# pedro-morgado/spatialaudiogen

Hardware: AMD Instinct MI355X
Metric: ambisonic seconds generated/sec (0.1 s windows, 224x448 video) (higher is better)
Workload: dtype f32 (fp32 in / out / accumulate; products on the 16-bit matrix cores with fp32-equivalent operand splits: two fp16 planes (3 products per multiply) for the ResNet trunk's 3x3 convs, whose operand ranges batch-norm bounds, three bf16 planes (6 products) elsewhere - measured against the fp64 oracle as

## Files before the change

spatialaudiogen_amd/csrc/igemm3.hip:

```cpp
#include "igemm3_common.h"

namespace sagen {

template <int BM, int BN, int WM, int WN, int KS, bool PRO>
__device__ __forceinline__ void igemm3_body(const IgemmDesc& d, const int z) {
    constexpr int MT = WM / 32, NT = WN / 32;
    constexpr int WAVES_N = BN / WN, WAVES_M = BM / WM;
    static_assert(WAVES_N * WAVES_M == 4, "4 waves per workgroup");
    constexpr int BK = 16;
    constexpr int NCH = BM >= 64 ? BM / 64 : 1;
    constexpr int NBC = (6 * BN + 255) / 256;
    constexpr int A_PL = BM * 8, B_PL = BN * 8;
    constexpr int SUB_F = 3 * A_PL + 3 * B_PL;
    constexpr int STAGE_F = KS * SUB_F;
    constexpr int NJOB = NBC + NBC + NCH + 3 * NCH;

    __shared__ __attribute__((aligned(16))) float smem[2 * STAGE_F];
    __shared__ RowInfo s_row[BM];
    __shared__ int s_tapb[MAX_TAPS];
    __shared__ __attribute__((aligned(16))) float s_bn[2][MAX_BN_C];

    const int tid = threadIdx.x;
    const int lane = tid & 63;
    const int wave = __builtin_amdgcn_readfirstlane(tid >> 6);
// ... 104 lines not shown
        if (!uni) bad |= (i_kok ^ 1u);
        bad_out = bad;
#ifndef SAGEN_ABLATE_A
        dst = bload16(x_rsrc, (a_voff[c] + i_tb) | (bad << 31));
#endif
    };
    auto load_b = [&](int c, f32x4& dst) {
#ifndef SAGEN_ABLATE_B
        dst = bload16(w_rsrc, (b_voff[c] + i_kbyte) | (i_past << 31));
#endif
    };
    auto store_b = [&](int c, const f32x4& src, float* st) {
#ifndef SAGEN_ABLATE_DSW
        if (NBC * 256 == 6 * BN || b_active[c]) *reinterpret_cast<f32x4*>(st + b_wofs[c]) = src;
#else
        asm volatile("" ::"v"(src));
#endif
    };
    float cv[KS][NCH][4];
    auto convert_job = [&](int ks, int c, int level, const f32x4& src, unsigned bad, int c0, float* st) {
        if (level == 0) {
            f32x4 v = src;
            if (PRO) {
                const int cc = c0 + 4 * kc4;
                const float4 sc = *reinterpret_cast<const float4*>(&s_bn[0][cc]);
                const float4 sh = *reinterpret_cast<const float4*>(&s_bn[1][cc]);
                const bool ok = bad == 0;
                v[0] = ok ? fmaxf(fmaf(v[0], sc.x, sh.x), 0.f) : 0.f;
                v[1] = ok ? fmaxf(fmaf(v[1], sc.y, sh.y), 0.f) : 0.f;
                v[2] = ok ? fmaxf(fmaf(v[2], sc.z, sh.z), 0.f) : 0.f;
                v[3] = ok ? fmaxf(fmaf(v[3], sc.w, sh.w), 0.f) : 0.f;
            }
            cv[ks][c][0] = v[0]; cv[ks][c][1] = v[1]; cv[ks][c][2] = v[2]; cv[ks][c][3] = v[3];
        }
        u32x2 pk;
        pk[0] = split_pair(cv[ks][c][0], cv[ks][c][1]);
        pk[1] = split_pair(cv[ks][c][2], cv[ks][c][3]);
#ifndef SAGEN_ABLATE_DSW
        if (a_active) *reinterpret_cast<u32x2*>(st + level * A_PL + a_wofs[c]) = pk;
#else
        asm volatile("" ::"v"(pk));
#endif
    };

    f32x16 acc[MT][NT];
#pragma unroll
    for (int i = 0; i < MT; ++i)
#pragma unroll
        for (int j = 0; j < NT; ++j)
#pragma unroll
            for (int e = 0; e < 16; ++e) acc[i][j][e] = 0.f;

    const int li = lane & 31, kk = lane >> 5;
    const int foff = 4 * (kk ^ ((li >> 3) & 1));

    auto side_job = [&](int job, int ks, auto pl_tag, float* st) {
        constexpr int PL = decltype(pl_tag)::value, PS = PL ^ 1;
        float* sub = st + ks * SUB_F;
        if (job < NBC) store_b(job, braw[PS][ks][job], sub);
        else if (job < 2 * NBC) load_b(job - NBC, braw[PL][ks][job - NBC]);
        else if (job < 2 * NBC + NCH) load_a(job - 2 * NBC, araw[PL][ks][job - 2 * NBC], abad[PL][ks][job - 2 * NBC]);
        else {
            const int cj = job - 2 * NBC - NCH, c = cj / 3;
            convert_job(ks, c, cj - 3 * c, araw[PS][ks][c], abad[PS][ks][c], ac0[PS][ks], sub);
        }
    };

#ifdef SAGEN_TRACE
    unsigned long long* trc = (d.trace && tile_m == d.trace_block && blockIdx.y == 0) ? (unsigned long long*)d.trace + (size_t)wave * 64 * 8 : nullptr;
#define TRC3(ph) do { if (trc && lane == 0 && t < 64) trc[t * 8 + (ph)] = __builtin_readcyclecounter(); } while (0)
#else
#define TRC3(ph) do { } while (0)
#endif
    constexpr int TA[6] = {0, 0, 1, 0, 2, 1}, TB[6] = {0, 1, 0, 2, 0, 1};
    const int nsteps = (ntiles + KS - 1) / KS;
#pragma unroll
    for (int ks = 0; ks < KS; ++ks) {
        begin_load(kc0 + ks, ac0[0][ks]);
#pragma unroll
        for (int c = 0; c < NBC; ++c) load_b(c, braw[0][ks][c]);
#pragma unroll
        for (int c = 0; c < NCH; ++c) load_a(c, araw[0][ks][c], abad[0][ks][c]);
    }
#pragma unroll
    for (int ks = 0; ks < KS; ++ks) {
        begin_load(kc0 + KS + ks, ac0[1][ks]);
#pragma unroll
        for (int c = 0; c < NBC; ++c) load_b(c, braw[1][ks][c]);
#pragma unroll
        for (int c = 0; c < NCH; ++c) load_a(c, araw[1][ks][c], abad[1][ks][c]);
    }
#pragma unroll
    for (int ks = 0; ks < KS; ++ks) {
#pragma unroll
        for (int c = 0; c < NBC; ++c) store_b(c, braw[0][ks][c], smem + ks * SUB_F);
#pragma unroll
        for (int c = 0; c < NCH; ++c)
#pragma unroll
            for (int lv = 0; lv < 3; ++lv) convert_job(ks, c, lv, araw[0][ks][c], abad[0][ks][c], ac0[0][ks], smem + ks * SUB_F);
    }
    lds_barrier();

    auto step = [&](auto parity, int t) {
        constexpr int P = decltype(parity)::value;
        const float* cur = smem + P * STAGE_F;
        float* nxt = smem + (P ^ 1) * STAGE_F;
            TRC3(0);
#pragma unroll
        for (int ks = 0; ks < KS; ++ks) {
            begin_load(kc0 + (t + 2) * KS + ks, ac0[P][ks]);
            bf16x8 aq[3][MT], bq[3][NT];
#pragma unroll
            for (int pl = 0; pl < 3; ++pl) {
#pragma unroll
                for (int i = 0; i < MT; ++i)
                    aq[pl][i] = *reinterpret_cast<const bf16x8*>(cur + ks * SUB_F + pl * A_PL + (wm * WM + i * 32 + li) * 8 + foff);
#pragma unroll
                for (int j = 0; j < NT; ++j)
                    bq[pl][j] = *reinterpret_cast<const bf16x8*>(cur + ks * SUB_F + 3 * A_PL + pl * B_PL + (wn * WN + j * 32 + li) * 8 + foff);
            }
#pragma unroll
            for (int tt = 0; tt < 6; ++tt)
#pragma unroll
                for (int i = 0; i < MT; ++i)
#pragma unroll
                    for (int j = 0; j < NT; ++j) {
#ifndef SAGEN_ABLATE_MFMA
                        acc[i][j] = __builtin_amdgcn_mfma_f32_32x32x16_bf16(aq[TA[tt]][i], bq[TB[tt]][j], acc[i][j], 0, 0, 0);
#else
                        asm volatile("" ::"v"(aq[TA[tt]][i]), "v"(bq[TB[tt]][j]));
#endif
                        constexpr int NM1 = 6 * MT * NT;
                        const int idx = (tt * MT + i) * NT + j;
#pragma unroll
                        for (int g = 0; g < NJOB; ++g)
                            if (idx == (g * NM1 / NJOB < NM1 ? g * NM1 / NJOB : NM1 - 1)) side_job(g, ks, std::integral_constant<int, P>{}, nxt);
#ifdef SAGEN_TRACE
                        if (ks == 0 && idx == 0) TRC3(1);
                        if (ks == KS - 1 && idx == NM1 - 1) TRC3(2);
#endif
                    }
        }
        asm volatile("s_waitcnt lgkmcnt(0)" ::: "memory");
        TRC3(3);
        lds_barrier();
        TRC3(4);
    };
    for (int t = 0; t < nsteps; t += 2) {
        step(std::integral_constant<int, 0>{}, t);
        if (t + 1 < nsteps) step(std::integral_constant<int, 1>{}, t + 1);
    }

    if (d.mm_out != nullptr) {
        if constexpr (BM <= 128 && BN <= 128 && WM * BN + 7 * 32 <= 2 * STAGE_F && !PRO)
            igemm_epilogue_maskmix<BM, BN, WM, WN, 2 * STAGE_F>(d, acc, smem, m0, n0, tid);
        return;
    }
    if (!igemm_epilogue_rows<BM, BN, WM, WN, 2 * STAGE_F>(d, acc, s_row, smem, n0, tid))
        igemm_epilogue<BM, BN, WM, WN>(d, acc, s_row, smem, m0, n0, z, tid);
}

template <int BM, int BN, int WM, int WN, int KS, bool PRO>
__global__ __launch_bounds__(256, 2) void igemm3_kernel(const IgemmDesc d_in) {
    IgemmDesc d = d_in;
    int z = blockIdx.z;
    if (d.grp.G > 1) {
        const int g = d.splitk == 1 ? z : z / d.splitk;
        z -= g * d.splitk;
        igemm_relocate(d, g);
    }
    igemm3_body<BM, BN, WM, WN, KS, PRO>(d, z);
}

template <int BM, int BN, int WM, int WN, int KS>
static int launch_cfg3(const IgemmDesc& d, hipStream_t s) {
    dim3 grid(cdiv(d.M, BM), cdiv(d.N, BN), d.splitk * d.grp.G);
    if (d.in_scale != nullptr || d.bn_in.acc != nullptr)
        hipLaunchKernelGGL((igemm3_kernel<BM, BN, WM, WN, KS, true>), grid, dim3(256), 0, s, d);
    else
        hipLaunchKernelGGL((igemm3_kernel<BM, BN, WM, WN, KS, false>), grid, dim3(256), 0, s, d);
    SAGEN_LAUNCH_CHECK();
    return SAGEN_OK;
}

int igemm3_dispatch(const IgemmDesc& d, IgemmTile tile, hipStream_t s) {
#define SAGEN_TILE_HAS_B3 ,
    switch (tile) {
        SAGEN_TILES(SAGEN_TILE_CASE)
        default: return igemm3dw_dispatch(d, tile, s);
    }
}

__global__ __launch_bounds__(256) void pack_split_kernel(const float* __restrict__ wp, long total, int N, int Kpad,
                                                         __bf16* __restrict__ w3) {
    const long idx = (long)blockIdx.x * 256 + threadIdx.x;
    if (idx >= total) return;
    const long n = idx / Kpad;
    const int k = (int)(idx - n * Kpad);
    const float v = wp[idx];
    const __bf16 h = (__bf16)v;
    const float r1 = v - (float)h;
    const __bf16 m = (__bf16)r1;
    const float r2 = r1 - (float)m;
    const long o = ((long)(k >> 4) * 3 * N + n) * 16 + (k & 15);
    w3[o] = h; w3[o + (long)N * 16] = m; w3[o + (long)N * 32] = (__bf16)r2;
}

int pack_split_launch(float* wp, int N, int Kpad, hipStream_t s) {
    const long total = (long)N * Kpad;
    hipLaunchKernelGGL(pack_split_kernel, dim3(cdiv(total, 256)), dim3(256), 0, s, wp, total, N, Kpad,
                       reinterpret_cast<__bf16*>(wp + total));
    SAGEN_LAUNCH_CHECK();
    return SAGEN_OK;
}

}
```

spatialaudiogen_amd/csrc/igemm_common.h:

```cpp
#pragma once
#include "kernels.h"
#include "h2_planes.h"

namespace sagen {

typedef float f32x16 __attribute__((ext_vector_type(16)));
constexpr int MAX_TAPS = 128;
constexpr unsigned OOB = 0x80000000u;
constexpr int MAX_BN_C = 512;

struct RowInfo {
    unsigned boff;
    unsigned nmlo, nmhi;
    int hrem, wrem;
    int pad;
    long rowoff;
};

__device__ __forceinline__ void dma16(__amdgpu_buffer_rsrc_t rsrc, float* lds, unsigned voff, unsigned soff) {
#if defined(__HIP_DEVICE_COMPILE__) && !defined(SAGEN_ABLATE_DMA)
    __builtin_amdgcn_raw_ptr_buffer_load_lds(rsrc, (__attribute__((address_space(3))) void*)lds, 16, voff, soff, 0, 0);
#endif
}

// ... 140 lines not shown
        __syncthreads();
        const int tile = (m0 / BM) * ((d.N + BN - 1) / BN) + n0 / BN;
        if (tid == 0) {
            const int t = __hip_atomic_fetch_add(&d.sk_ticket[tile], 1, __ATOMIC_RELAXED, __HIP_MEMORY_SCOPE_AGENT);
            s_last = t == d.splitk - 1;
            if (s_last) __hip_atomic_store(&d.sk_ticket[tile], 0, __ATOMIC_RELAXED, __HIP_MEMORY_SCOPE_AGENT);
        }
        __syncthreads();
        if (s_last) {
            constexpr int C4 = BN / 4;
            auto ld4 = [](const float* q) {
                return make_float4(__hip_atomic_load(q, __ATOMIC_RELAXED, __HIP_MEMORY_SCOPE_AGENT), __hip_atomic_load(q + 1, __ATOMIC_RELAXED, __HIP_MEMORY_SCOPE_AGENT),
                                   __hip_atomic_load(q + 2, __ATOMIC_RELAXED, __HIP_MEMORY_SCOPE_AGENT), __hip_atomic_load(q + 3, __ATOMIC_RELAXED, __HIP_MEMORY_SCOPE_AGENT));
            };
            const long MN = (long)d.M * d.N;
            for (int idx = tid; idx < BM * C4; idx += 256) {
                const int r = idx / C4, m = m0 + r, n = n0 + 4 * (idx - r * C4);
                if (m >= d.M || n >= d.N) continue;
                const float* p = d.splitk_ws + (long)m * d.N + n;
                float4 v = make_float4(0.f, 0.f, 0.f, 0.f);
                int zz = 0;
                for (; zz + 4 <= d.splitk; zz += 4, p += 4 * MN) {
                    const float4 t0 = ld4(p), t1 = ld4(p + MN);
                    const float4 t2 = ld4(p + 2 * MN), t3 = ld4(p + 3 * MN);
                    v.x += (t0.x + t1.x) + (t2.x + t3.x); v.y += (t0.y + t1.y) + (t2.y + t3.y);
                    v.z += (t0.z + t1.z) + (t2.z + t3.z); v.w += (t0.w + t1.w) + (t2.w + t3.w);
                }
                for (; zz < d.splitk; ++zz, p += MN) {
                    const float4 t = ld4(p);
                    v.x += t.x; v.y += t.y; v.z += t.z; v.w += t.w;
                }
                if (d.bias) { v.x += d.bias[n]; v.y += d.bias[n + 1]; v.z += d.bias[n + 2]; v.w += d.bias[n + 3]; }
                if (d.relu_out) { v.x = fmaxf(v.x, 0.f); v.y = fmaxf(v.y, 0.f); v.z = fmaxf(v.z, 0.f); v.w = fmaxf(v.w, 0.f); }
                for (int rr = 0; rr < d.sk_rep; ++rr) *reinterpret_cast<float4*>(d.y + ((long)m * d.sk_rep + rr) * d.ldy + n) = v;
            }
        }
    }
    if (d.stats != nullptr) {
        __syncthreads();
#pragma unroll
        for (int j = 0; j < NT; ++j) {
            float s = wave_xor_add<32>(csum[j]);
            float q = wave_xor_add<32>(csq[j]);
            if (kk == 0) {
                const int col = wn * WN + j * 32 + li;
                red[(0 * WAVES_M + wm) * BN + col] = s;
                red[(1 * WAVES_M + wm) * BN + col] = q;
            }
        }
        __syncthreads();
        for (int t = tid; t < 2 * BN; t += 256) {
            const int which = t / BN, col = t - which * BN;
            const int n = n0 + col;
            if (n < d.N) {
                float s = 0.f;
#pragma unroll
                for (int w2 = 0; w2 < WAVES_M; ++w2) s += red[(which * WAVES_M + w2) * BN + col];
                atomicAdd(&d.stats[(long)which * d.N + n], (double)s);
            }
        }
    }
}

template <int BM, int BN, int WM, int WN, int CAP>
__device__ __forceinline__ bool igemm_epilogue_rows(const IgemmDesc& d, f32x16 (&acc)[WM / 32][WN / 32], const RowInfo* s_row,
                                                    float* red, int n0, int tid) {
    constexpr int MT = WM / 32, NT = WN / 32;
    constexpr int WAVES_N = BN / WN, WAVES_M = BM / WM;
    constexpr int TPR = BN / 4, RPP = 256 / TPR;
    if constexpr (WM % RPP != 0 || WM * BN + 2 * RPP * BN > CAP) {
        return false;
    } else {
        if (d.dsh * d.dsw != 1 || d.splitk_ws != nullptr) return false;
        constexpr int NPASS = WM / RPP;
        const int lane = tid & 63;
        const int wave = __builtin_amdgcn_readfirstlane(tid >> 6);
        const int wm = wave / WAVES_N, wn = wave % WAVES_N;
        const int li = lane & 31, kk = lane >> 5;
        float* const tile = red;
        float* const part_sums = red + WM * BN;
        const int c4 = tid % TPR, rg = tid / TPR;
        const int n = n0 + 4 * c4;
        const bool vec_ok = n + 3 < d.N && (d.ldy % 4 == 0) && ((reinterpret_cast<uintptr_t>(d.y) & 15) == 0);
        float4 bias = make_float4(0.f, 0.f, 0.f, 0.f);
        if (d.bias) {
            bias.x = n < d.N ? d.bias[n] : 0.f; bias.y = n + 1 < d.N ? d.bias[n + 1] : 0.f;
            bias.z = n + 2 < d.N ? d.bias[n + 2] : 0.f; bias.w = n + 3 < d.N ? d.bias[n + 3] : 0.f;
        }
        float4 cs = make_float4(0.f, 0.f, 0.f, 0.f), cq = make_float4(0.f, 0.f, 0.f, 0.f);
        float amax = 0.f;
#pragma unroll
        for (int part = 0; part < WAVES_M; ++part) {
            if (wm == part) {
#pragma unroll
                for (int i = 0; i < MT; ++i)
#pragma unroll
                    for (int j = 0; j < NT; ++j)
#pragma unroll
                        for (int e = 0; e < 16; ++e)
                            tile[(i * 32 + (e & 3) + 8 * (e >> 2) + 4 * kk) * BN + wn * WN + j * 32 + li] = acc[i][j][e];
            }
            __syncthreads();
            long ro[NPASS];
            bool ok[NPASS];
            float4 tv[NPASS];
#pragma unroll
            for (int k = 0; k < NPASS; ++k) {
                const RowInfo& ri = s_row[part * WM + rg + k * RPP];
                ok[k] = ri.hrem > 0 && ri.wrem > 0;
                ro[k] = ri.rowoff;
            }
#pragma unroll
            for (int k = 0; k < NPASS; ++k) tv[k] = *reinterpret_cast<const float4*>(tile + (rg + k * RPP) * BN + 4 * c4);
#pragma unroll
            for (int k = 0; k < NPASS; ++k) {
                if (!ok[k]) continue;
                float4 v = tv[k];
                cs.x += v.x; cs.y += v.y; cs.z += v.z; cs.w += v.w;
                cq.x += v.x * v.x; cq.y += v.y * v.y; cq.z += v.z * v.z; cq.w += v.w * v.w;
                v.x += bias.x; v.y += bias.y; v.z += bias.z; v.w += bias.w;
                if (d.relu_out) { v.x = fmaxf(v.x, 0.f); v.y = fmaxf(v.y, 0.f); v.z = fmaxf(v.z, 0.f); v.w = fmaxf(v.w, 0.f); }
                float* dst = d.y + ro[k] + n;
                if (vec_ok) *reinterpret_cast<float4*>(dst) = v;
                else {
                    if (n < d.N) dst[0] = v.x;
                    if (n + 1 < d.N) dst[1] = v.y;
                    if (n + 2 < d.N) dst[2] = v.z;
                    if (n + 3 < d.N) dst[3] = v.w;
                }
                amax = fmaxf(amax, fmaxf(fmaxf(n < d.N ? fabsf(v.x) : 0.f, n + 1 < d.N ? fabsf(v.y) : 0.f),
                                         fmaxf(n + 2 < d.N ? fabsf(v.z) : 0.f, n + 3 < d.N ? fabsf(v.w) : 0.f)));
            }
            if (part + 1 < WAVES_M) __syncthreads();
        }
        if (d.amax_out != nullptr) igemm_publish_amax(d.amax_out, amax);
        if (d.stats != nullptr) {
            *reinterpret_cast<float4*>(part_sums + (0 * RPP + rg) * BN + 4 * c4) = cs;
            *reinterpret_cast<float4*>(part_sums + (1 * RPP + rg) * BN + 4 * c4) = cq;
            __syncthreads();
            for (int t = tid; t < 2 * BN; t += 256) {
                const int which = t / BN, col = t - which * BN;
                if (n0 + col < d.N) {
                    float sum = 0.f;
#pragma unroll
                    for (int g = 0; g < RPP; ++g) sum += part_sums[(which * RPP + g) * BN + col];
                    atomicAdd(&d.stats[(long)which * d.N + n0 + col], (double)sum);
                }
            }
        }
        return true;
    }
}

template <int BM, int BN, int WM, int WN, int CAP>
__device__ __forceinline__ void igemm_epilogue_maskmix(const IgemmDesc& d, f32x16 (&acc)[WM / 32][WN / 32], float* red, int m0, int n0,
                                                       int tid) {
    constexpr int NTR = 32;
    constexpr int MT = WM / 32, NT = WN / 32;
    constexpr int WAVES_N = BN / WN, WAVES_M = BM / WM;
    constexpr int SUBS = BN / NTR, ITEMS = WM * SUBS * 2;
    static_assert(WM * BN + 7 * NTR <= CAP, "mask-mix staging must fit the tile ring");
    static_assert(ITEMS % 2 == 0 && BN % NTR == 0, "whole output pixels per tile");
    float* const tile = red;
    float* const wl = red + WM * BN;
    float* const bs = wl + 6 * NTR;
    const int lane = tid & 63;
    const int wave = __builtin_amdgcn_readfirstlane(tid >> 6);
    const int wm = wave / WAVES_N, wn = wave % WAVES_N;
    const int li = lane & 31, kk = lane >> 5;
    const int HgWg = d.Hg * d.Wg;
    const int b = m0 / HgWg;
    const int rem = m0 - b * HgWg;
    const int ia = rem / d.Wg;
    const int q0 = d.g_w0 + rem - ia * d.Wg;
    const int dswC = d.dsw * NTR;
    const int ry = n0 / dswC, rx0 = (n0 - ry * dswC) / NTR;
    const int y = (d.g_h0 + ia) * d.dsh + ry, fi = y - d.mm_row0;
    if (m0 >= d.M || y >= d.Hlim || fi < 0 || fi >= d.mm_nf) return;
    const int f = d.mm_f_lo + fi;
    const int n_lo = max(256 * f - 1216, 0), n_hi = min(256 * f - 1216 + 1023, 4799);
    const int s_lo = n_lo / 1600, s_hi = n_hi / 1600;
    const bool two = s_hi != s_lo;
    for (int i = tid; i < 6 * NTR; i += 256) {
        const int j = i % NTR, o = (i / NTR) % 3, si = i / (3 * NTR);
        wl[i] = d.mm_coeffs[(((long)b * 3 + (si ? s_hi : s_lo)) * 3 + o) * (NTR + 1) + j];
    }
    if (tid < NTR) bs[tid] = d.bias ? d.bias[tid] : 0.f;
#pragma unroll
    for (int part = 0; part < WAVES_M; ++part) {
        if (wm == part) {
#pragma unroll
            for (int i = 0; i < MT; ++i)
#pragma unroll
                for (int j = 0; j < NT; ++j)
#pragma unroll
                    for (int e = 0; e < 16; ++e)
                        tile[(i * 32 + (e & 3) + 8 * (e >> 2) + 4 * kk) * BN + wn * WN + j * 32 + li] = acc[i][j][e];
        }
        __syncthreads();
        for (int item = tid; item < ITEMS; item += 256) {
            const int half = item & 1, sub = (item >> 1) % SUBS, r = (item >> 1) / SUBS;
            float e[6] = {0.f, 0.f, 0.f, 0.f, 0.f, 0.f};
#pragma unroll
            for (int q4 = 0; q4 < 4; ++q4) {
                const float4 v = *reinterpret_cast<const float4*>(tile + r * BN + sub * NTR + half * 16 + 4 * q4);
                const float vv[4] = {v.x, v.y, v.z, v.w};
#pragma unroll
                for (int u = 0; u < 4; ++u) {
                    const int j = half * 16 + 4 * q4 + u;
                    const float sg = __builtin_amdgcn_rcpf(1.f + __builtin_amdgcn_exp2f(-1.4426950408889634f * (vv[u] + bs[j])));
#pragma unroll
                    for (int o = 0; o < 3; ++o) {
                        e[o] = fmaf(wl[o * NTR + j], sg, e[o]);
                        if (two) e[3 + o] = fmaf(wl[(3 + o) * NTR + j], sg, e[3 + o]);
                    }
                }
            }
#pragma unroll
            for (int c = 0; c < 6; ++c) e[c] = wave_xor_add<1>(e[c]);
            const int row = part * WM + r;
            const int x = (q0 + row) * d.dsw + rx0 + sub;
            if (half == 0 && m0 + row < d.M && x < d.Wlim) {
                float4* dst = reinterpret_cast<float4*>(d.mm_out + (((long)b * d.mm_nf + fi) * d.Wlim + x) * 8);
                dst[0] = make_float4(e[0], e[1], e[2], e[3]);
                dst[1] = make_float4(e[4], e[5], 0.f, 0.f);
            }
        }
        if (part + 1 < WAVES_M) __syncthreads();
    }
}

}
```

spatialaudiogen_amd/csrc/stem8.hip:

```cpp
#include "igemm3_common.h"
#include "h2_planes.h"

namespace sagen {

constexpr int S8_PH = 8, S8_PW = 7;
constexpr int S8_RH = 2 * S8_PH + 1;
constexpr int S8_RW = 2 * S8_PW + 1;
constexpr int S8_M = S8_RH * S8_RW;
__device__ __forceinline__ int s8_slot(int m) { return m ^ ((m >> 1) & 1); }
constexpr int S8_UH = 229, S8_UW = 456;
constexpr int S8_NH = 32;
constexpr int S8_W_BYTES = 14 * 3 * S8_NH * 32;
constexpr int S8_CT_BYTES = 256 * S8_NH * 4;
constexpr int S8_THREADS = 512;
constexpr int S8_LDS = S8_W_BYTES + S8_CT_BYTES + 2 * 8 * S8_NH * 4 + S8_NH * 4;
typedef _Float16 f16x8s __attribute__((ext_vector_type(8)));

size_t stem8_plane_bytes(int B) { return (size_t)B * S8_UH * S8_UW * 8; }

template <bool HALF>
__global__ __launch_bounds__(256) void stem8_prep_kernel(const unsigned char* __restrict__ x_, u32x2* __restrict__ plane_, int B,
                                                         float* __restrict__ zero_ptr_, long zero_n, const GroupInfo gi) {
    const unsigned char* __restrict__ x = x_ + (size_t)blockIdx.z * ((size_t)B * 224 * 448 * 3);
    u32x2* __restrict__ plane = SAGEN_GRP(plane_);
    float* __restrict__ zero_ptr = SAGEN_GRP(zero_ptr_);
    const long total = (long)B * S8_UH * S8_UW;
    for (long i = (long)blockIdx.x * 256 + threadIdx.x; i < zero_n; i += (long)gridDim.x * 256) zero_ptr[i] = 0.f;
    auto conv = [](unsigned u) -> unsigned {
        return HALF ? (unsigned)__builtin_bit_cast(unsigned short, (_Float16)(float)((int)u - 128))
                    : __builtin_bit_cast(unsigned, (float)((int)u - 128)) >> 16;
    };
    constexpr int QW = S8_UW / 4;
    static_assert(S8_UW % 4 == 0, "plane rows are whole quads");
    const long nquad = (long)B * S8_UH * QW;
    const unsigned border = HALF ? 0xB800u : 0xBF00u;
    for (long iq = (long)blockIdx.x * 256 + threadIdx.x; iq < nquad; iq += (long)gridDim.x * 256) {
        long p = iq;
        const int q = (int)(p % QW); p /= QW;
        const int h = (int)(p % S8_UH) - 2;
        const int b = (int)(p / S8_UH);
        const int w0 = 4 * q - 2;
        u32x2 o[4];
        if ((unsigned)h < 224u && w0 >= 0 && w0 + 3 < 448) {
            const long ob = (((long)b * 224 + h) * 448 + w0) * 3;
            constexpr unsigned sh = 2;
            const unsigned* src = reinterpret_cast<const unsigned*>(x + (ob - sh));
            const unsigned d[4] = {src[0], src[1], src[2], src[3]};
            unsigned by[12];
#pragma unroll
            for (int k = 0; k < 12; ++k) by[k] = (d[(sh + k) >> 2] >> (8 * ((sh + k) & 3))) & 0xffu;
#pragma unroll
            for (int k = 0; k < 4; ++k) o[k] = u32x2{conv(by[3 * k]) | (conv(by[3 * k + 1]) << 16), conv(by[3 * k + 2])};
        } else {
#pragma unroll
            for (int k = 0; k < 4; ++k) {
                const int w = w0 + k;
                unsigned c0 = border, c1 = border, c2 = border;
                if ((unsigned)h < 224u && (unsigned)w < 448u) {
                    const unsigned char* src = x + (((long)b * 224 + h) * 448 + w) * 3;
                    c0 = conv(src[0]); c1 = conv(src[1]); c2 = conv(src[2]);
                }
                o[k] = u32x2{c0 | (c1 << 16), c2};
            }
        }
        u32x4* dst = reinterpret_cast<u32x4*>(plane + iq * 4);
        dst[0] = u32x4{o[0][0], o[0][1], o[1][0], o[1][1]};
        dst[1] = u32x4{o[2][0], o[2][1], o[3][0], o[3][1]};
    }
    (void)total;
}

template <int OUT, int MODE = 0>
__global__ __launch_bounds__(S8_THREADS, 2) void stem8pool_kernel(const char* __restrict__ plane_, const float* __restrict__ wf32,
                                                                  const char* __restrict__ wplanes, const float* __restrict__ gamma,
                                                                  float* __restrict__ pooled_, double* __restrict__ stats_, int B,
                                                                  long plane_stride, const float* __restrict__ a_inv_, const float* __restrict__ w_inv_,
                                                                  float* __restrict__ raw2_, const GroupInfo gi) {
    const char* __restrict__ plane = SAGEN_GRP(plane_);
    float* __restrict__ pooled = SAGEN_GRP(pooled_);
    double* __restrict__ stats = SAGEN_GRP(stats_);
    const float* __restrict__ a_inv = SAGEN_GRP(a_inv_);
    const float* __restrict__ w_inv = SAGEN_GRP(w_inv_);
    float* __restrict__ raw2 = SAGEN_GRP(raw2_);
    constexpr bool F16 = MODE != 0;
    constexpr int NPLA = MODE == 1 ? 2 : 1, NPLW = MODE == 0 ? 3 : 2;
    constexpr int W_BYTES = 14 * NPLW * S8_NH * 32;
    extern __shared__ __attribute__((aligned(16))) char smem[];
    char* const wl = smem;
    char* const pa = smem + S8_W_BYTES;
    float* const ct = reinterpret_cast<float*>(smem + S8_W_BYTES);
    float* const red = reinterpret_cast<float*>(smem + S8_W_BYTES + S8_CT_BYTES);
    float* const cb = reinterpret_cast<float*>(smem + S8_W_BYTES + S8_CT_BYTES + 2 * 8 * S8_NH * 4);
    const int tid = threadIdx.x;
    const int lane = tid & 63;
    const int wave = __builtin_amdgcn_readfirstlane(tid >> 6);
    const int li = lane & 31, g = lane >> 5;
    const int nh = blockIdx.x & 1;
    const int wg = blockIdx.x >> 1, nwg = gridDim.x >> 1;

    for (int i = tid; i < W_BYTES / 16; i += S8_THREADS) {
        const int row = i >> 1, hf = i & 1;
        const int kp = row >> 5, n = row & 31;
        reinterpret_cast<f32x4*>(wl)[i] = *reinterpret_cast<const f32x4*>(wplanes + ((long)(kp * 64 + nh * 32 + n) * 32 + 16 * (hf ^ ((n >> 3) & 1))));
    }
    if (tid < S8_NH) {
        double s = 0.0;
        if (MODE != 1)
            for (int k = 0; k < 224; ++k) s += (double)wf32[(nh * S8_NH + tid) * 224 + k];
        cb[tid] = (float)(s * (0.5 / 255.0));
    }
    const float osc = MODE == 1 ? a_inv[0] * w_inv[0] : (MODE == 2 ? w_inv[0] * (1.f / 255.f) : 1.f / 255.f);
    const int pch4 = tid & 7;
    bool use_min[4];
#pragma unroll
    for (int k = 0; k < 4; ++k) use_min[k] = OUT == 1 ? false : gamma[nh * S8_NH + 4 * pch4 + k] < 0.f;
    constexpr bool SGN = OUT == 0;
    float sgn4[4];
#pragma unroll
    for (int k = 0; k < 4; ++k) sgn4[k] = (SGN && use_min[k]) ? -1.f : 1.f;
    const float sgn_l = (SGN && gamma[nh * S8_NH + li] < 0.f) ? -1.f : 1.f;
    int poff[9];
    {
        const int p = tid >> 3;
        const int pr_l = p / S8_PW, pc_l = p - pr_l * S8_PW;
#pragma unroll
        for (int dr = 0; dr < 3; ++dr)
#pragma unroll
            for (int dc = 0; dc < 3; ++dc) poff[dr * 3 + dc] = s8_slot((2 * pr_l + dr) * S8_RW + 2 * pc_l + dc) * S8_NH + 4 * pch4;
    }
    unsigned own = 0;
#pragma unroll
    for (int e = 0; e < 16; ++e) {
        const int m = wave * 32 + (e & 3) + 8 * (e >> 2) + 4 * g;
        const int r = m / S8_RW, c = m - r * S8_RW;
        if (m < S8_M && r < 2 * S8_PH && c < 2 * S8_PW) own |= 1u << e;
    }
    float ssum = 0.f, ssq = 0.f;
    __syncthreads();
    const float cbl = cb[li] * sgn_l;
    const float osc_l = osc * sgn_l;

    const int npatch = B * 7 * 16;
    constexpr int PROWS = 2 * (S8_RH - 1) + 7, PCH = (2 * (S8_RW - 1) + 8) / 2;
    constexpr int NCHUNK = PROWS * PCH;
    constexpr int PATCH_BYTES = NCHUNK * 16;
    static_assert(NCHUNK <= 2 * S8_THREADS && NPLA * PATCH_BYTES <= S8_CT_BYTES, "patch staging");
    const int ck0 = tid, ck1 = tid + S8_THREADS;
    const int cr0 = ck0 / PCH, cc0 = ck0 - cr0 * PCH, cr1 = ck1 / PCH, cc1 = ck1 - cr1 * PCH;
    auto patch_src = [&](int patch, int crow, int ccol) {
        const int b = patch / 112, rem = patch - b * 112;
        const int pr = rem >> 4, pc = rem & 15;
        const int row = min(2 * 16 * pr + crow, S8_UH - 1);
        return plane + (((long)b * S8_UH + row) * S8_UW + 2 * 14 * pc) * 8 + ccol * 16;
    };
    f32x4 ld0[NPLA], ld1[NPLA];
#pragma unroll
    for (int p = 0; p < NPLA; ++p) {
        ld0[p] = f32x4{0.f, 0.f, 0.f, 0.f}; ld1[p] = ld0[p];
        if (wg < npatch) {
            ld0[p] = *reinterpret_cast<const f32x4*>(patch_src(wg, cr0, cc0) + p * plane_stride);
            if (ck1 < NCHUNK) ld1[p] = *reinterpret_cast<const f32x4*>(patch_src(wg, cr1, cc1) + p * plane_stride);
        }
    }
    int aoff;
    {
        const int m = wave * 32 + li;
        int r = m / S8_RW, c = m - r * S8_RW;
        if (m >= S8_M) { r = 0; c = 0; }
        aoff = ((2 * r) * (2 * PCH) + 2 * c + 2 * g) * 8;
    }
    for (int patch = wg; patch < npatch; patch += nwg) {
        const int b = patch / 112, rem = patch - b * 112;
        const int pr = rem >> 4, pc = rem & 15;
        const int R0 = 16 * pr, C0 = 14 * pc;
#pragma unroll
        for (int p = 0; p < NPLA; ++p) {
            reinterpret_cast<f32x4*>(pa + p * PATCH_BYTES)[ck0] = ld0[p];
            if (ck1 < NCHUNK) reinterpret_cast<f32x4*>(pa + p * PATCH_BYTES)[ck1] = ld1[p];
        }
        __syncthreads();
        const int next_patch = patch + nwg;
        if (next_patch < npatch) {
#pragma unroll
            for (int p = 0; p < NPLA; ++p) {
                ld0[p] = *reinterpret_cast<const f32x4*>(patch_src(next_patch, cr0, cc0) + p * plane_stride);
                if (ck1 < NCHUNK) ld1[p] = *reinterpret_cast<const f32x4*>(patch_src(next_patch, cr1, cc1) + p * plane_stride);
            }
        }
        f32x16 acc[2];
#pragma unroll
        for (int j = 0; j < 2; ++j)
#pragma unroll
            for (int e = 0; e < 16; ++e) acc[j][e] = 0.f;
#pragma unroll
        for (int ks = 0; ks < 14; ++ks) {
            bf16x8 fa[NPLA], fb[NPLW];
#pragma unroll
            for (int p = 0; p < NPLA; ++p) fa[p] = *reinterpret_cast<const bf16x8*>(pa + p * PATCH_BYTES + aoff + ((ks >> 1) * (2 * PCH) + (ks & 1) * 4) * 8);
#pragma unroll
            for (int pl = 0; pl < NPLW; ++pl) fb[pl] = *reinterpret_cast<const bf16x8*>(wl + ((ks * NPLW + pl) * S8_NH + li) * 32 + 16 * (g ^ ((li >> 3) & 1)));
            const int a = ks & 1;
            if constexpr (MODE == 2) {
                acc[a] = __builtin_amdgcn_mfma_f32_32x32x16_f16(__builtin_bit_cast(f16x8s, fa[0]), __builtin_bit_cast(f16x8s, fb[1]), acc[a], 0, 0, 0);
                acc[a ^ 1] = __builtin_amdgcn_mfma_f32_32x32x16_f16(__builtin_bit_cast(f16x8s, fa[0]), __builtin_bit_cast(f16x8s, fb[0]), acc[a ^ 1], 0, 0, 0);
            } else if constexpr (F16) {
                acc[a] = __builtin_amdgcn_mfma_f32_32x32x16_f16(__builtin_bit_cast(f16x8s, fa[NPLA - 1]), __builtin_bit_cast(f16x8s, fb[0]), acc[a], 0, 0, 0);
                acc[a ^ 1] = __builtin_amdgcn_mfma_f32_32x32x16_f16(__builtin_bit_cast(f16x8s, fa[0]), __builtin_bit_cast(f16x8s, fb[NPLW - 1]), acc[a ^ 1], 0, 0, 0);
                acc[a] = __builtin_amdgcn_mfma_f32_32x32x16_f16(__builtin_bit_cast(f16x8s, fa[0]), __builtin_bit_cast(f16x8s, fb[0]), acc[a], 0, 0, 0);
            } else {
                acc[a] = __builtin_amdgcn_mfma_f32_32x32x16_bf16(fa[0], fb[NPLW - 1], acc[a], 0, 0, 0);
                acc[a ^ 1] = __builtin_amdgcn_mfma_f32_32x32x16_bf16(fa[0], fb[1], acc[a ^ 1], 0, 0, 0);
                acc[a] = __builtin_amdgcn_mfma_f32_32x32x16_bf16(fa[0], fb[0], acc[a], 0, 0, 0);
            }
        }
        __syncthreads();
#pragma unroll
        for (int e = 0; e < 16; ++e) {
            const float v = fmaf(acc[0][e] + acc[1][e], osc_l, cbl);
            ct[s8_slot(wave * 32 + (e & 3) + 8 * (e >> 2) + 4 * g) * S8_NH + li] = v;
            const float vo = ((own >> e) & 1u) ? v : 0.f;
            ssum += vo;
            ssq = fmaf(vo, vo, ssq);
        }
        __syncthreads();
        if (OUT >= 1) {
            float* const raw = OUT == 2 ? raw2 : pooled;
            for (int it = tid; it < 2 * S8_PH * 2 * S8_PW * 8; it += S8_THREADS) {
                const int p = it >> 3, q4 = it & 7;
                const int r = p / (2 * S8_PW), cc = p - r * (2 * S8_PW);
                *reinterpret_cast<float4*>(raw + (((long)b * 112 + R0 + r) * 224 + C0 + cc) * 64 + nh * S8_NH + 4 * q4) =
                    *reinterpret_cast<const float4*>(ct + s8_slot(r * S8_RW + cc) * S8_NH + 4 * q4);
            }
        }
        if (OUT != 1 && tid < S8_PH * S8_PW * 8) {
            const int p = tid >> 3;
            const int pr_l = p / S8_PW, pc_l = p - pr_l * S8_PW;
            float4 v[9];
            if (pr < 6 && pc < 15) {
#pragma unroll
                for (int k = 0; k < 9; ++k) v[k] = *reinterpret_cast<const float4*>(ct + poff[k]);
            } else {
#pragma unroll
                for (int dr = 0; dr < 3; ++dr)
#pragma unroll
                    for (int dc = 0; dc < 3; ++dc) {
                        const int rr = (R0 + 2 * pr_l + dr >= 112) ? 2 * pr_l : 2 * pr_l + dr;
                        const int cc = (C0 + 2 * pc_l + dc >= 224) ? 2 * pc_l : 2 * pc_l + dc;
                        v[dr * 3 + dc] = *reinterpret_cast<const float4*>(ct + s8_slot(rr * S8_RW + cc) * S8_NH + 4 * pch4);
                    }
            }
            float4 ext = v[0];
            if constexpr (SGN) {
#pragma unroll
                for (int k = 1; k < 9; ++k) {
                    ext.x = fmaxf(ext.x, v[k].x); ext.y = fmaxf(ext.y, v[k].y); ext.z = fmaxf(ext.z, v[k].z); ext.w = fmaxf(ext.w, v[k].w);
                }
                ext.x *= sgn4[0]; ext.y *= sgn4[1]; ext.z *= sgn4[2]; ext.w *= sgn4[3];
            } else {
#pragma unroll
                for (int k = 1; k < 9; ++k) {
                    ext.x = use_min[0] ? fminf(ext.x, v[k].x) : fmaxf(ext.x, v[k].x); ext.y = use_min[1] ? fminf(ext.y, v[k].y) : fmaxf(ext.y, v[k].y);
                    ext.z = use_min[2] ? fminf(ext.z, v[k].z) : fmaxf(ext.z, v[k].z); ext.w = use_min[3] ? fminf(ext.w, v[k].w) : fmaxf(ext.w, v[k].w);
                }
            }
            *reinterpret_cast<float4*>(pooled + (((long)b * 56 + 8 * pr + pr_l) * 112 + 7 * pc + pc_l) * 64 + nh * S8_NH + 4 * pch4) = ext;
        }
        __syncthreads();
    }
    ssum *= sgn_l;
    ssum = wave_xor_add<32>(ssum);
    ssq = wave_xor_add<32>(ssq);
    if (g == 0) {
        red[(0 * 8 + wave) * S8_NH + li] = ssum;
        red[(1 * 8 + wave) * S8_NH + li] = ssq;
    }
    __syncthreads();
    if (tid < 2 * S8_NH) {
        const int which = tid >> 5, ch = tid & 31;
        float s = 0.f;
#pragma unroll
        for (int k = 0; k < 8; ++k) s += red[(which * 8 + k) * S8_NH + ch];
        atomicAdd(&stats[which * 64 + nh * S8_NH + ch], (double)s);
    }
}

int stem8_prep_launch(const unsigned char* x, void* plane, int B, hipStream_t s, float* zero_ptr, long zero_n, int half) {
    if (!x || !plane) return fail(SAGEN_ERR_NULL, "stem8_prep: null argument");
    if (((uintptr_t)x % 4) || ((uintptr_t)plane % 16)) return fail(SAGEN_ERR_UNSUPPORTED, "stem8_prep: the frames must be 4-byte aligned, the plane 16-byte aligned");
    const long total = (long)B * S8_UH * S8_UW / 4;
    const int grid = (int)std::min<long>(cdiv(total, 256), 256L * 16);
    const GroupInfo gi = cur_group();
    if (half) hipLaunchKernelGGL(stem8_prep_kernel<true>, dim3(grid, 1, gi.G), dim3(256), 0, s, x, reinterpret_cast<u32x2*>(plane), B, zero_ptr, zero_ptr ? zero_n : 0L, gi);
    else hipLaunchKernelGGL(stem8_prep_kernel<false>, dim3(grid, 1, gi.G), dim3(256), 0, s, x, reinterpret_cast<u32x2*>(plane), B, zero_ptr, zero_ptr ? zero_n : 0L, gi);
    SAGEN_LAUNCH_CHECK();
    return SAGEN_OK;
}

int stem8pool_launch(const void* plane, const float* wp, const float* gamma, float* pooled, double* stats, int B, hipStream_t s) {
    if (!plane || !wp || !gamma || !pooled || !stats) return fail(SAGEN_ERR_NULL, "stem8pool: null argument");
    static bool attr_set = false;
    if (!attr_set) {
        SAGEN_HIP_CHECK(hipFuncSetAttribute(reinterpret_cast<const void*>(stem8pool_kernel<0>), hipFuncAttributeMaxDynamicSharedMemorySize, S8_LDS));
        attr_set = true;
    }
    const char* planes = reinterpret_cast<const char*>(wp + 64 * 224);
    const int npatch = B * 7 * 16;
    hipLaunchKernelGGL(stem8pool_kernel<0>, dim3(2 * std::min(npatch, 256), 1, cur_group().G), dim3(S8_THREADS), S8_LDS, s, reinterpret_cast<const char*>(plane), wp, planes, gamma,
                       pooled, stats, B, 0L, (const float*)nullptr, (const float*)nullptr, (float*)nullptr, cur_group());
    SAGEN_LAUNCH_CHECK();
    return SAGEN_OK;
}

int stem8pool_h2_launch(const void* plane, const float* wp, const void* wh2, const float* w_inv, const float* gamma, float* pooled, double* stats, int B,
                        hipStream_t s) {
    if (!plane || !wp || !wh2 || !w_inv || !gamma || !pooled || !stats) return fail(SAGEN_ERR_NULL, "stem8pool_h2: null argument");
    static bool attr_set = false;
    if (!attr_set) {
        SAGEN_HIP_CHECK(hipFuncSetAttribute(reinterpret_cast<const void*>(stem8pool_kernel<0, 2>), hipFuncAttributeMaxDynamicSharedMemorySize, S8_LDS));
        attr_set = true;
    }
    const int npatch = B * 7 * 16;
    hipLaunchKernelGGL((stem8pool_kernel<0, 2>), dim3(2 * std::min(npatch, 256), 1, cur_group().G), dim3(S8_THREADS), S8_LDS, s, reinterpret_cast<const char*>(plane), wp,
                       reinterpret_cast<const char*>(wh2), gamma, pooled, stats, B, 0L, (const float*)nullptr, w_inv, (float*)nullptr, cur_group());
    SAGEN_LAUNCH_CHECK();
    return SAGEN_OK;
}

int stem8raw_launch(const void* plane, const float* wp, float* y0, double* stats, int B, hipStream_t s) {
    if (!plane || !wp || !y0 || !stats) return fail(SAGEN_ERR_NULL, "stem8raw: null argument");
    static bool attr_set = false;
    if (!attr_set) {
        SAGEN_HIP_CHECK(hipFuncSetAttribute(reinterpret_cast<const void*>(stem8pool_kernel<1>), hipFuncAttributeMaxDynamicSharedMemorySize, S8_LDS));
        attr_set = true;
    }
    const char* planes = reinterpret_cast<const char*>(wp + 64 * 224);
    const int npatch = B * 7 * 16;
    hipLaunchKernelGGL(stem8pool_kernel<1>, dim3(2 * std::min(npatch, 256), 1, cur_group().G), dim3(S8_THREADS), S8_LDS, s, reinterpret_cast<const char*>(plane), wp, planes,
                       (const float*)nullptr, y0, stats, B, 0L, (const float*)nullptr, (const float*)nullptr, (float*)nullptr, cur_group());
    SAGEN_LAUNCH_CHECK();
    return SAGEN_OK;
}

int stem8rawpool_launch(const void* plane, const float* wp, const float* gamma, float* y0, float* pooled, double* stats, int B, hipStream_t s) {
    if (!plane || !wp || !gamma || !y0 || !pooled || !stats) return fail(SAGEN_ERR_NULL, "stem8rawpool: null argument");
    static bool attr_set = false;
    if (!attr_set) {
        SAGEN_HIP_CHECK(hipFuncSetAttribute(reinterpret_cast<const void*>(stem8pool_kernel<2>), hipFuncAttributeMaxDynamicSharedMemorySize, S8_LDS));
        attr_set = true;
    }
    const char* planes = reinterpret_cast<const char*>(wp + 64 * 224);
    const int npatch = B * 7 * 16;
    hipLaunchKernelGGL(stem8pool_kernel<2>, dim3(2 * std::min(npatch, 256), 1, cur_group().G), dim3(S8_THREADS), S8_LDS, s, reinterpret_cast<const char*>(plane), wp, planes,
                       gamma, pooled, stats, B, 0L, (const float*)nullptr, (const float*)nullptr, y0, cur_group());
    SAGEN_LAUNCH_CHECK();
    return SAGEN_OK;
}

constexpr int S16_PARTS = 1024;
__global__ __launch_bounds__(256) void stem16_amax_kernel(const float* __restrict__ x_, long n4, float* __restrict__ part_, float* __restrict__ zero_ptr_, long zero_n, const GroupInfo gi) {
    const float* __restrict__ x = x_ + (size_t)blockIdx.z * (size_t)n4 * 4;
    float* __restrict__ part = SAGEN_GRP(part_);
    float* __restrict__ zero_ptr = SAGEN_GRP(zero_ptr_);
    for (long i = (long)blockIdx.x * 256 + threadIdx.x; i < zero_n; i += (long)gridDim.x * 256) zero_ptr[i] = 0.f;
    float m = 0.f;
    for (long i = (long)blockIdx.x * 256 + threadIdx.x; i < n4; i += (long)gridDim.x * 256) {
        const float4 v = reinterpret_cast<const float4*>(x)[i];
        m = fmaxf(m, fmaxf(fmaxf(fabsf(v.x), fabsf(v.y)), fmaxf(fabsf(v.z), fabsf(v.w))));
    }
    m = wave_max_f(m);
    __shared__ float s_m[4];
    if ((threadIdx.x & 63) == 0) s_m[threadIdx.x >> 6] = m;
    __syncthreads();
    if (threadIdx.x == 0) part[blockIdx.x] = fmaxf(fmaxf(s_m[0], s_m[1]), fmaxf(s_m[2], s_m[3]));
}
__global__ __launch_bounds__(256) void stem16_prep_kernel(const float* __restrict__ x_, u32x2* __restrict__ hi_, u32x2* __restrict__ lo_, int B,
                                                          const float* __restrict__ part_, float* __restrict__ a_inv_, const GroupInfo gi) {
    const float* __restrict__ x = x_ + (size_t)blockIdx.z * ((size_t)B * 224 * 448 * 3);
    u32x2* __restrict__ hi = SAGEN_GRP(hi_);
    u32x2* __restrict__ lo = SAGEN_GRP(lo_);
    const float* __restrict__ part = SAGEN_GRP(part_);
    float* __restrict__ a_inv = SAGEN_GRP(a_inv_);
    float m = 0.f;
    for (int i = threadIdx.x & 63; i < S16_PARTS; i += 64) m = fmaxf(m, part[i]);
    m = wave_max_f(m);
    const float sa = h2_scale_of_bound(m);
    if (blockIdx.x == 0 && threadIdx.x == 0) a_inv[0] = 1.f / sa;
    const long total = (long)B * S8_UH * S8_UW;
    for (long i = (long)blockIdx.x * 256 + threadIdx.x; i < total; i += (long)gridDim.x * 256) {
        long p = i;
        const int w = (int)(p % S8_UW) - 2; p /= S8_UW;
        const int h = (int)(p % S8_UH) - 2;
        const int b = (int)(p / S8_UH);
        unsigned short hh[3] = {0, 0, 0}, ll[3] = {0, 0, 0};
        if ((unsigned)h < 224u && (unsigned)w < 448u) {
            const float* src = x + (((long)b * 224 + h) * 448 + w) * 3;
#pragma unroll
            for (int c = 0; c < 3; ++c) {
                const float v = src[c] * sa;
                const _Float16 a = __builtin_isfinite(v) ? (_Float16)v : __builtin_bit_cast(_Float16, (unsigned short)0x7e00);
                const _Float16 r = __builtin_isfinite(v) ? (_Float16)(v - (float)a) : (_Float16)0.f;
                hh[c] = __builtin_bit_cast(unsigned short, a); ll[c] = __builtin_bit_cast(unsigned short, r);
            }
        }
        hi[i] = u32x2{(unsigned)hh[0] | ((unsigned)hh[1] << 16), (unsigned)hh[2]};
        lo[i] = u32x2{(unsigned)ll[0] | ((unsigned)ll[1] << 16), (unsigned)ll[2]};
    }
}

int stem16_prep_launch(const float* x, void* planes, float* part, float* a_inv, int B, hipStream_t s, float* zero_ptr, long zero_n) {
    if (!x || !planes || !part || !a_inv) return fail(SAGEN_ERR_NULL, "stem16_prep: null argument");
    const long n = (long)B * 224 * 448 * 3;
    if (n % 4 || ((uintptr_t)x % 16)) return fail(SAGEN_ERR_UNSUPPORTED, "stem16_prep: the frames must be 16-byte aligned");
    const GroupInfo gi = cur_group();
    hipLaunchKernelGGL(stem16_amax_kernel, dim3(S16_PARTS, 1, gi.G), dim3(256), 0, s, x, n / 4, part, zero_ptr, zero_ptr ? zero_n : 0L, gi);
    const long total = (long)B * S8_UH * S8_UW;
    char* p = reinterpret_cast<char*>(planes);
    hipLaunchKernelGGL(stem16_prep_kernel, dim3((int)std::min<long>(cdiv(total, 256), 256L * 16), 1, gi.G), dim3(256), 0, s, x, reinterpret_cast<u32x2*>(p),
                       reinterpret_cast<u32x2*>(p + stem8_plane_bytes(B)), B, part, a_inv, gi);
    SAGEN_LAUNCH_CHECK();
    return SAGEN_OK;
}

int stem16pool_launch(const void* planes, const void* wh2, const float* gamma, float* pooled, double* stats, const float* a_inv, const float* w_inv,
                      int B, hipStream_t s) {
    if (!planes || !wh2 || !gamma || !pooled || !stats || !a_inv || !w_inv) return fail(SAGEN_ERR_NULL, "stem16pool: null argument");
    static bool attr_set = false;
    if (!attr_set) {
        SAGEN_HIP_CHECK(hipFuncSetAttribute(reinterpret_cast<const void*>(stem8pool_kernel<0, 1>), hipFuncAttributeMaxDynamicSharedMemorySize, S8_LDS));
        attr_set = true;
    }
    const int npatch = B * 7 * 16;
    hipLaunchKernelGGL((stem8pool_kernel<0, 1>), dim3(2 * std::min(npatch, 256), 1, cur_group().G), dim3(S8_THREADS), S8_LDS, s, reinterpret_cast<const char*>(planes),
                       (const float*)nullptr, reinterpret_cast<const char*>(wh2), gamma, pooled, stats, B, (long)stem8_plane_bytes(B), a_inv, w_inv, (float*)nullptr, cur_group());
    SAGEN_LAUNCH_CHECK();
    return SAGEN_OK;
}

}
```

Baseline: 3281.

## Make mask-mix epilogue wave-private and process two quads per thread in stem prep

The mask-mix epilogue now gives each wave its own swizzled LDS staging tile and holds the coefficient and bias tables in registers. This replaces the workgroup-wide __syncthreads loop over wave rows with wave-local barriers, removing cross-wave serialization and LDS bank conflicts. Separately, the stem8 prep kernel handles two pixel quads per thread using 32-bit index math, with loads issued ahead of the conversions. The cost is higher register pressure from the per-lane tables and a new frame-count limit check.

```diff
diff --git a/spatialaudiogen_amd/csrc/igemm3.hip b/spatialaudiogen_amd/csrc/igemm3.hip
--- a/spatialaudiogen_amd/csrc/igemm3.hip
+++ b/spatialaudiogen_amd/csrc/igemm3.hip
@@ -280,7 +280,7 @@
     }
 
     if (d.mm_out != nullptr) {
-        if constexpr (BM <= 128 && BN <= 128 && WM * BN + 7 * 32 <= 2 * STAGE_F && !PRO)
+        if constexpr (BM <= 128 && BN <= 128 && igemm_maskmix_fits<WM, WN, 2 * STAGE_F>() && !PRO)
             igemm_epilogue_maskmix<BM, BN, WM, WN, 2 * STAGE_F>(d, acc, smem, m0, n0, tid);
         return;
     }
diff --git a/spatialaudiogen_amd/csrc/igemm_common.h b/spatialaudiogen_amd/csrc/igemm_common.h
--- a/spatialaudiogen_amd/csrc/igemm_common.h
+++ b/spatialaudiogen_amd/csrc/igemm_common.h
@@ -316,22 +316,26 @@
     }
 }
 
+template <int WM, int WN, int CAP>
+constexpr bool igemm_maskmix_fits() { return 4 * WM * 32 <= CAP; }
+
 template <int BM, int BN, int WM, int WN, int CAP>
 __device__ __forceinline__ void igemm_epilogue_maskmix(const IgemmDesc& d, f32x16 (&acc)[WM / 32][WN / 32], float* red, int m0, int n0,
                                                        int tid) {
     constexpr int NTR = 32;
-    constexpr int MT = WM / 32, NT = WN / 32;
-    constexpr int WAVES_N = BN / WN, WAVES_M = BM / WM;
-    constexpr int SUBS = BN / NTR, ITEMS = WM * SUBS * 2;
-    static_assert(WM * BN + 7 * NTR <= CAP, "mask-mix staging must fit the tile ring");
-    static_assert(ITEMS % 2 == 0 && BN % NTR == 0, "whole output pixels per tile");
-    float* const tile = red;
-    float* const wl = red + WM * BN;
-    float* const bs = wl + 6 * NTR;
+    constexpr int MT = WM / 32;
+    constexpr int WAVES_N = BN / WN;
+    constexpr int CW = (WN >= 64 && 4 * WM * 64 <= CAP) ? 64 : 32;
+    constexpr int NCP = WN / CW, JB = CW / 32;
+    constexpr int SUBS = CW / NTR, ITEMS = WM * SUBS * 2;
+    constexpr int RSH = CW == 64 ? 0 : 1;
+    static_assert(4 * WM * CW <= CAP, "mask-mix staging must fit the tile ring");
+    static_assert(ITEMS % 64 == 0 && WN % CW == 0 && BN % NTR == 0, "whole output pixels per wave");
     const int lane = tid & 63;
     const int wave = __builtin_amdgcn_readfirstlane(tid >> 6);
     const int wm = wave / WAVES_N, wn = wave % WAVES_N;
     const int li = lane & 31, kk = lane >> 5;
+    float* const tile = red + wave * (WM * CW);
     const int HgWg = d.Hg * d.Wg;
     const int b = m0 / HgWg;
     const int rem = m0 - b * HgWg;
@@ -345,53 +349,73 @@
     const int n_lo = max(256 * f - 1216, 0), n_hi = min(256 * f - 1216 + 1023, 4799);
     const int s_lo = n_lo / 1600, s_hi = n_hi / 1600;
     const bool two = s_hi != s_lo;
-    for (int i = tid; i < 6 * NTR; i += 256) {
-        const int j = i % NTR, o = (i / NTR) % 3, si = i / (3 * NTR);
-        wl[i] = d.mm_coeffs[(((long)b * 3 + (si ? s_hi : s_lo)) * 3 + o) * (NTR + 1) + j];
-    }
-    if (tid < NTR) bs[tid] = d.bias ? d.bias[tid] : 0.f;
-#pragma unroll
-    for (int part = 0; part < WAVES_M; ++part) {
-        if (wm == part) {
-#pragma unroll
-            for (int i = 0; i < MT; ++i)
-#pragma unroll
-                for (int j = 0; j < NT; ++j)
-#pragma unroll
-                    for (int e = 0; e < 16; ++e)
-                        tile[(i * 32 + (e & 3) + 8 * (e >> 2) + 4 * kk) * BN + wn * WN + j * 32 + li] = acc[i][j][e];
-        }
-        __syncthreads();
-        for (int item = tid; item < ITEMS; item += 256) {
-            const int half = item & 1, sub = (item >> 1) % SUBS, r = (item >> 1) / SUBS;
+    const int half = lane & 1;
+    float wv[2][3][16], bs[16];
+    auto load_tables = [&]() {
+#pragma unroll
+        for (int si = 0; si < 2; ++si)
+#pragma unroll
+            for (int o = 0; o < 3; ++o) {
+                const float* src = d.mm_coeffs + (((long)b * 3 + (si ? s_hi : s_lo)) * 3 + o) * (NTR + 1) + half * 16;
+#pragma unroll
+                for (int u = 0; u < 16; ++u) wv[si][o][u] = (si == 0 || two) ? src[u] : 0.f;
+            }
+#pragma unroll
+        for (int u = 0; u < 16; ++u) bs[u] = d.bias ? d.bias[half * 16 + u] : 0.f;
+    };
+#pragma unroll
+    for (int cp = 0; cp < NCP; ++cp) {
+#pragma unroll
+        for (int i = 0; i < MT; ++i)
+#pragma unroll
+            for (int jb = 0; jb < JB; ++jb)
+#pragma unroll
+                for (int e = 0; e < 16; ++e) {
+                    const int r = i * 32 + (e & 3) + 8 * (e >> 2) + 4 * kk;
+                    tile[r * CW + ((jb * 32 + li) ^ (((r >> RSH) & 3) << 2))] = acc[i][cp * JB + jb][e];
+                }
+        if (cp == 0) load_tables();
+        __builtin_amdgcn_fence(__ATOMIC_ACQ_REL, "wavefront");
+        __builtin_amdgcn_wave_barrier();
+#pragma unroll
+        for (int it = 0; it < ITEMS / 64; ++it) {
+            const int item = it * 64 + lane;
+            const int sub = (item >> 1) % SUBS, r = (item >> 1) / SUBS;
+            const float* const src = tile + r * CW + sub * NTR + half * 16;
+            const int swz = (r >> RSH) & 3;
+            float4 v[4];
+#pragma unroll
+            for (int q4 = 0; q4 < 4; ++q4) v[q4] = *reinterpret_cast<const float4*>(src + 4 * (q4 ^ swz));
             float e[6] = {0.f, 0.f, 0.f, 0.f, 0.f, 0.f};
 #pragma unroll
             for (int q4 = 0; q4 < 4; ++q4) {
-                const float4 v = *reinterpret_cast<const float4*>(tile + r * BN + sub * NTR + half * 16 + 4 * q4);
-                const float vv[4] = {v.x, v.y, v.z, v.w};
+                const float vv[4] = {v[q4].x, v[q4].y, v[q4].z, v[q4].w};
 #pragma unroll
                 for (int u = 0; u < 4; ++u) {
-                    const int j = half * 16 + 4 * q4 + u;
+                    const int j = 4 * q4 + u;
                     const float sg = __builtin_amdgcn_rcpf(1.f + __builtin_amdgcn_exp2f(-1.4426950408889634f * (vv[u] + bs[j])));
 #pragma unroll
                     for (int o = 0; o < 3; ++o) {
-                        e[o] = fmaf(wl[o * NTR + j], sg, e[o]);
-                        if (two) e[3 + o] = fmaf(wl[(3 + o) * NTR + j], sg, e[3 + o]);
+                        e[o] = fmaf(wv[0][o][j], sg, e[o]);
+                        if (two) e[3 + o] = fmaf(wv[1][o][j], sg, e[3 + o]);
                     }
                 }
             }
 #pragma unroll
             for (int c = 0; c < 6; ++c) e[c] = wave_xor_add<1>(e[c]);
-            const int row = part * WM + r;
-            const int x = (q0 + row) * d.dsw + rx0 + sub;
+            const int row = wm * WM + r;
+            const int x = (q0 + row) * d.dsw + rx0 + (wn * WN + cp * CW) / NTR + sub;
             if (half == 0 && m0 + row < d.M && x < d.Wlim) {
                 float4* dst = reinterpret_cast<float4*>(d.mm_out + (((long)b * d.mm_nf + fi) * d.Wlim + x) * 8);
                 dst[0] = make_float4(e[0], e[1], e[2], e[3]);
                 dst[1] = make_float4(e[4], e[5], 0.f, 0.f);
             }
         }
-        if (part + 1 < WAVES_M) __syncthreads();
-    }
-}
-
-}
+        if (cp + 1 < NCP) {
+            __builtin_amdgcn_fence(__ATOMIC_ACQ_REL, "wavefront");
+            __builtin_amdgcn_wave_barrier();
+        }
+    }
+}
+
+}
diff --git a/spatialaudiogen_amd/csrc/stem8.hip b/spatialaudiogen_amd/csrc/stem8.hip
--- a/spatialaudiogen_amd/csrc/stem8.hip
+++ b/spatialaudiogen_amd/csrc/stem8.hip
@@ -30,42 +30,53 @@
         return HALF ? (unsigned)__builtin_bit_cast(unsigned short, (_Float16)(float)((int)u - 128))
                     : __builtin_bit_cast(unsigned, (float)((int)u - 128)) >> 16;
     };
-    constexpr int QW = S8_UW / 4;
-    static_assert(S8_UW % 4 == 0, "plane rows are whole quads");
-    const long nquad = (long)B * S8_UH * QW;
+    constexpr int QW = S8_UW / 4, NQ = 2, PW = QW / NQ;
+    static_assert(S8_UW % 4 == 0 && QW % NQ == 0, "plane rows are whole quad pairs");
+    const unsigned nunit = (unsigned)B * S8_UH * PW;
     const unsigned border = HALF ? 0xB800u : 0xBF00u;
-    for (long iq = (long)blockIdx.x * 256 + threadIdx.x; iq < nquad; iq += (long)gridDim.x * 256) {
-        long p = iq;
-        const int q = (int)(p % QW); p /= QW;
-        const int h = (int)(p % S8_UH) - 2;
-        const int b = (int)(p / S8_UH);
-        const int w0 = 4 * q - 2;
-        u32x2 o[4];
-        if ((unsigned)h < 224u && w0 >= 0 && w0 + 3 < 448) {
+    for (unsigned iu = blockIdx.x * 256 + threadIdx.x; iu < nunit; iu += gridDim.x * 256) {
+        const unsigned rowi = iu / PW;
+        const int q0 = NQ * (int)(iu - rowi * PW);
+        const int b = (int)(rowi / S8_UH);
+        const int h = (int)(rowi - (unsigned)b * S8_UH) - 2;
+        bool fast[NQ];
+        unsigned d[NQ][4];
+#pragma unroll
+        for (int t = 0; t < NQ; ++t) {
+            const int w0 = 4 * (q0 + t) - 2;
+            fast[t] = (unsigned)h < 224u && w0 >= 0 && w0 + 3 < 448;
             const long ob = (((long)b * 224 + h) * 448 + w0) * 3;
-            constexpr unsigned sh = 2;
-            const unsigned* src = reinterpret_cast<const unsigned*>(x + (ob - sh));
-            const unsigned d[4] = {src[0], src[1], src[2], src[3]};
-            unsigned by[12];
-#pragma unroll
-            for (int k = 0; k < 12; ++k) by[k] = (d[(sh + k) >> 2] >> (8 * ((sh + k) & 3))) & 0xffu;
-#pragma unroll
-            for (int k = 0; k < 4; ++k) o[k] = u32x2{conv(by[3 * k]) | (conv(by[3 * k + 1]) << 16), conv(by[3 * k + 2])};
-        } else {
-#pragma unroll
-            for (int k = 0; k < 4; ++k) {
-                const int w = w0 + k;
-                unsigned c0 = border, c1 = border, c2 = border;
-                if ((unsigned)h < 224u && (unsigned)w < 448u) {
-                    const unsigned char* src = x + (((long)b * 224 + h) * 448 + w) * 3;
-                    c0 = conv(src[0]); c1 = conv(src[1]); c2 = conv(src[2]);
+            const unsigned* src = reinterpret_cast<const unsigned*>(x + (fast[t] ? ob - 2 : 0L));
+#pragma unroll
+            for (int k = 0; k < 4; ++k) d[t][k] = src[k];
+        }
+        u32x4* dst = reinterpret_cast<u32x4*>(plane + (size_t)iu * (4 * NQ));
+#pragma unroll
+        for (int t = 0; t < NQ; ++t) {
+            const int w0 = 4 * (q0 + t) - 2;
+            u32x2 o[4];
+            if (fast[t]) {
+                constexpr unsigned sh = 2;
+                unsigned by[12];
+#pragma unroll
+                for (int k = 0; k < 12; ++k) by[k] = (d[t][(sh + k) >> 2] >> (8 * ((sh + k) & 3))) & 0xffu;
+#pragma unroll
+                for (int k = 0; k < 4; ++k) o[k] = u32x2{conv(by[3 * k]) | (conv(by[3 * k + 1]) << 16), conv(by[3 * k + 2])};
+            } else {
+#pragma unroll
+                for (int k = 0; k < 4; ++k) {
+                    const int w = w0 + k;
+                    unsigned c0 = border, c1 = border, c2 = border;
+                    if ((unsigned)h < 224u && (unsigned)w < 448u) {
+                        const unsigned char* src = x + (((long)b * 224 + h) * 448 + w) * 3;
+                        c0 = conv(src[0]); c1 = conv(src[1]); c2 = conv(src[2]);
+                    }
+                    o[k] = u32x2{c0 | (c1 << 16), c2};
                 }
-                o[k] = u32x2{c0 | (c1 << 16), c2};
-            }
-        }
-        u32x4* dst = reinterpret_cast<u32x4*>(plane + iq * 4);
-        dst[0] = u32x4{o[0][0], o[0][1], o[1][0], o[1][1]};
-        dst[1] = u32x4{o[2][0], o[2][1], o[3][0], o[3][1]};
+            }
+            dst[2 * t] = u32x4{o[0][0], o[0][1], o[1][0], o[1][1]};
+            dst[2 * t + 1] = u32x4{o[2][0], o[2][1], o[3][0], o[3][1]};
+        }
     }
     (void)total;
 }
@@ -287,8 +298,9 @@
 int stem8_prep_launch(const unsigned char* x, void* plane, int B, hipStream_t s, float* zero_ptr, long zero_n, int half) {
     if (!x || !plane) return fail(SAGEN_ERR_NULL, "stem8_prep: null argument");
     if (((uintptr_t)x % 4) || ((uintptr_t)plane % 16)) return fail(SAGEN_ERR_UNSUPPORTED, "stem8_prep: the frames must be 4-byte aligned, the plane 16-byte aligned");
-    const long total = (long)B * S8_UH * S8_UW / 4;
-    const int grid = (int)std::min<long>(cdiv(total, 256), 256L * 16);
+    const long total = (long)B * S8_UH * S8_UW / 8;
+    if (total >= (1L << 31)) return fail(SAGEN_ERR_UNSUPPORTED, "stem8_prep: too many frames for 32-bit index arithmetic");
+    const int grid = (int)std::min<long>(cdiv(total, 256), 256L * 8);
     const GroupInfo gi = cur_group();
     if (half) hipLaunchKernelGGL(stem8_prep_kernel<true>, dim3(grid, 1, gi.G), dim3(256), 0, s, x, reinterpret_cast<u32x2*>(plane), B, zero_ptr, zero_ptr ? zero_n : 0L, gi);
     else hipLaunchKernelGGL(stem8_prep_kernel<false>, dim3(grid, 1, gi.G), dim3(256), 0, s, x, reinterpret_cast<u32x2*>(plane), B, zero_ptr, zero_ptr ? zero_n : 0L, gi);
```

New measurement: 3286 (median of 4 runs). No clear change (+0.2%).
